# Chlumsky/msdfgen

Hardware: AMD Instinct MI355X
Metric: MSDF glyphs/sec (64x64, fp32) (higher is better)
Workload: dtype f64

## Files before the change

### msdfgen_amd/csrc/msdf_ec_fast.hpp

```cpp
#pragma once

#include "msdf_ec.hpp"

namespace msdfhip {

enum { EC_DEFER = 0x80 };

enum { EC_V_ERROR = 1,
       EC_V_CHECK = 2,
       EC_V_COND = 4,
       EC_V_HELD = 8 };
enum { EC_ORDER_EAGER = 0, EC_ORDER_LAZY = 1, EC_ORDER_LAZY_HELD = 2 };

MSDF_HD bool ecHasBasePass(const EcParams &p) { return p.distanceCheck == EC_DO_NOT_CHECK || (p.distanceCheck == EC_CHECK_AT_EDGE && p.mode != EC_MODE_EDGE_ONLY); }
MSDF_HD bool ecHasShapePass(const EcParams &p) { return p.distanceCheck == EC_ALWAYS_CHECK || p.distanceCheck == EC_CHECK_AT_EDGE; }
MSDF_HD bool ecLazyProtect(const EcParams &p) { return p.mode == EC_MODE_EDGE_PRIORITY && p.distanceCheck == EC_CHECK_AT_EDGE; }

struct FastCtx {
    double span;
    bool p1;
    bool pShape;
    bool basePass, shapePass;
    int order;
};

MSDF_HD int rangeTest2(const FastCtx &c, double at, double bt, double xt, float am, float bm, float xm) {
    const bool inversion = (am > .5f && bm > .5f && xm <= .5f) || (am < .5f && bm < .5f && xm >= .5f);
    const bool outside = medianf(am, bm, xm) != xm;
    const bool candBase = c.basePass && (inversion || (!c.p1 && outside));
    const bool candShape = c.shapePass && (inversion || (!c.pShape && outside));
    const bool candCond = c.order != EC_ORDER_EAGER && !inversion && outside;
    if (!(candBase || candShape || candCond))
        return 0;
    const double axSpan = (xt-at)*c.span, bxSpan = (bt-xt)*c.span;
    const int f = (xm >= am-axSpan && xm <= am+axSpan && xm >= bm-bxSpan && xm <= bm+bxSpan) ? 1 : 3;
    return (candBase ? f : 0)|(candShape ? f<<2 : 0)|(candCond && f == 3 ? 16 : 0);
}

MSDF_HD int judge(int flags) {
    const int cond = (flags&16) ? EC_V_COND : 0;
    if (flags&2)
        return EC_V_ERROR|cond;
    const int fs = (flags>>2)&3;
    if (fs&1)
        return ((fs&2) ? EC_V_ERROR : EC_V_CHECK)|cond;
    return cond;
}

MSDF_HD bool quadraticMayHaveRootInRange(double a, double b, double c) {
    if (a == 0 || fabs(b) > 1e12*fabs(a))
        return true;
    const double lo = .005, hi = .995;
    const double mag = fabs(a)+fabs(b)+fabs(c);
    const double eps = 1e-9*mag;
    const double flo = (a*lo+b)*lo+c, fhi = (a*hi+b)*hi+c;
    if (!(flo > eps && fhi > eps) && !(flo < -eps && fhi < -eps))
        return true;
    const double s = flo > 0 ? 1. : -1.;
    const double as = a*s, bs = b*s, cs = c*s;
    if (as <= 0)
        return false;
    if (!(-bs > 2*as*lo*(1-1e-9) && -bs < 2*as*hi*(1+1e-9)))
        return false;
    return !(4*as*cs-bs*bs > 1e-9*mag*mag);
}

MSDF_HD bool bernsteinMayHaveRoot(float dA, float dBC, float dD) {
    const float m = fmaxf(fmaxf(fabsf(dA), fabsf(dBC)), fabsf(dD));
    const float eps = 1e-5f*m;
    const float h = .5f*dBC;
    return !((dA > eps && h > eps && dD > eps) || (dA < -eps && h < -eps && dD < -eps));
}

MSDF_HD bool edgeBetweenTexelsChannelFast(const float *a, const float *b, int channel) {
    const double n = a[channel]-.5;
    const double d = a[channel]-b[channel];
    if (!((n > 0 && d > 0 && n < d) || (n < 0 && d < 0 && n > d)))
        return false;
    const double t = n/d;
    if (t > 0 && t < 1) {
        float c[3] = { mixf(a[0], b[0], t), mixf(a[1], b[1], t), mixf(a[2], b[2], t) };
        return medianf(c[0], c[1], c[2]) == c[channel];
    }
    return false;
}

MSDF_HD int edgeBetweenTexelsFast(const float *a, const float *b) {
    return 1*(int) edgeBetweenTexelsChannelFast(a, b, 0)+2*(int) edgeBetweenTexelsChannelFast(a, b, 1)+4*(int) edgeBetweenTexelsChannelFast(a, b, 2);
}

template <class Sink>
MSDF_HD int diagonalPairFast(const FastCtx &cx, float am, float dm, const float *a, const float *l, const float *q,
                             float dA, float dBC, float dD, float l0, float q0, float l1, float q1, Sink &sink) {
    const double qa = dD-dBC+dA, qb = dBC-dA-dA, qc = dA;
    if (!quadraticMayHaveRootInRange(qa, qb, qc))
        return 0;
    double t[2];
    const int solutions = solveQuadratic(t, qa, qb, qc);
    int verdict = 0;
    for (int i = 0; i < solutions; ++i) {
        if (t[i] > MSDF_ARTIFACT_T_EPSILON && t[i] < 1-MSDF_ARTIFACT_T_EPSILON) {
            const float xm = interpolatedMedianQuad(a, l, q, t[i]);
            int rangeFlags = rangeTest2(cx, 0, 1, t[i], am, dm, xm);
            const double tEx0 = -.5*l0/q0, tEx1 = -.5*l1/q1;
            if (tEx0 > 0 && tEx0 < 1) {
                double tEnd0 = 0, tEnd1 = 1;
                float em0 = am, em1 = dm;
                const float ex = interpolatedMedianQuad(a, l, q, tEx0);
                if (tEx0 > t[i])
                    tEnd1 = tEx0, em1 = ex;
                else
                    tEnd0 = tEx0, em0 = ex;
                rangeFlags |= rangeTest2(cx, tEnd0, tEnd1, t[i], em0, em1, xm);
            }
            if (tEx1 > 0 && tEx1 < 1) {
                double tEnd0 = 0, tEnd1 = 1;
                float em0 = am, em1 = dm;
                const float ex = interpolatedMedianQuad(a, l, q, tEx1);
                if (tEx1 > t[i])
                    tEnd1 = tEx1, em1 = ex;
                else
                    tEnd0 = tEx1, em0 = ex;
                rangeFlags |= rangeTest2(cx, tEnd0, tEnd1, t[i], em0, em1, xm);
            }
            const int v = judge(rangeFlags);
            verdict |= v;
            if (v&EC_V_CHECK) {
                const bool held = (verdict&EC_V_COND) != 0;
                if (held)
                    verdict |= EC_V_HELD;
                if (held == (cx.order == EC_ORDER_LAZY_HELD))
                    sink(t[i]);
            }
            if (verdict&EC_V_ERROR)
                return verdict;
        }
    }
    return verdict;
}

struct Neighbourhood {
    float v[3][3][3];
    float dev[3][3];
    unsigned valid;
};

MSDF_HD float ecTexelDeviation(const float *t) { return fabsf(medianf(t[0], t[1], t[2])-.5f); }

MSDF_HD void loadNeighbourhood(Neighbourhood &nb, const SdfView &sdf, int x, int yn) {
    nb.valid = 0;
    MSDF_UNROLL
    for (int dy = -1; dy <= 1; ++dy) {
        MSDF_UNROLL
        for (int dx = -1; dx <= 1; ++dx) {
            const int nx = x+dx, ny = yn+dy;
            const bool in = nx >= 0 && ny >= 0 && nx < sdf.w && ny < sdf.h;
            const float *t = sdf.native(in ? nx : x, in ? ny : yn);
            nb.v[dy+1][dx+1][0] = t[0], nb.v[dy+1][dx+1][1] = t[1], nb.v[dy+1][dx+1][2] = t[2];
            nb.dev[dy+1][dx+1] = ecTexelDeviation(t);
            if (in)
                nb.valid |= 1u<<((dy+1)*3+(dx+1));
        }
    }
}

template <class Emit>
MSDF_HD void texelProtectPairs(const Neighbourhood &nb, const EcParams &p, Emit &emit) {
    const float sdev = nb.dev[1][1];
    MSDF_UNROLL
    for (int dy = -1; dy <= 1; ++dy) {
        MSDF_UNROLL
        for (int dx = -1; dx <= 1; ++dx) {
            if (!dx && !dy)
                continue;
            if (!(nb.valid&(1u<<((dy+1)*3+(dx+1)))))
                continue;
            const float radius = dy == 0 ? p.radiusH : dx == 0 ? p.radiusV : p.radiusD;
            const float odev = nb.dev[dy+1][dx+1];
            const bool selfIsA = dy > 0 || (dy == 0 && dx > 0);
            const float sum = selfIsA ? sdev+odev : odev+sdev;
            if (sum < radius)
                emit((dy+1)*3+(dx+1));
        }
    }
}

MSDF_HD bool evaluateProtectPair(const float *self, const float *other, int m) {
    const int dy = m/3-1, dx = m%3-1;
    const bool selfIsA = dy > 0 || (dy == 0 && dx > 0);
    const int mask = selfIsA ? edgeBetweenTexelsFast(self, other) : edgeBetweenTexelsFast(other, self);
    return extremeChannelInMask(self, medianf(self[0], self[1], self[2]), mask);
}

MSDF_HD bool protectedByEdgesNb(const Neighbourhood &nb, const EcParams &p) {
    struct Items {
        unsigned char m[8];
        int n;
        MSDF_HD void operator()(int mm) { m[n++] = (unsigned char) mm; }
    } items;
    items.n = 0;
    texelProtectPairs(nb, p, items);
    for (int i = 0; i < items.n; ++i)
        if (evaluateProtectPair(nb.v[1][1], nb.v[items.m[i]/3][items.m[i]%3], items.m[i]))
            return true;
    return false;
}

MSDF_HD int ecNeighbourDx(int k) { return k < 4 ? (k == 0 ? -1 : k == 2 ? 1 : 0) : ((k&1) ? 1 : -1); }
MSDF_HD int ecNeighbourDy(int k) { return k < 4 ? (k == 1 ? -1 : k == 3 ? 1 : 0) : ((k&2) ? 1 : -1); }

template <class Emit>
MSDF_HD void texelCandidatePairs(const Neighbourhood &nb, Emit &emit) {
    const float *c = nb.v[1][1];
    const float cdev = nb.dev[1][1];
    MSDF_UNROLL
    for (int k = 0; k < 4; ++k) {
        const int dx = k == 0 ? -1 : k == 2 ? 1 : 0, dy = k == 1 ? -1 : k == 3 ? 1 : 0;
        if (!(nb.valid&(1u<<((dy+1)*3+(dx+1)))))
            continue;
        const float *b = nb.v[dy+1][dx+1];
        if (!(cdev >= nb.dev[dy+1][dx+1]))
            continue;
        MSDF_UNROLL
        for (int j = 0; j < 3; ++j) {
            const int i0 = j, i1 = j == 2 ? 0 : j+1;
            const float dA = c[i1]-c[i0], dB = b[i1]-b[i0];
            if ((dA > 0 && dB < 0) || (dA < 0 && dB > 0))
                emit(k, j);
        }
    }
    MSDF_UNROLL
    for (int k = 4; k < 8; ++k) {
        const int dx = (k&1) ? 1 : -1, dy = (k&2) ? 1 : -1;
        if (!(nb.valid&(1u<<((dy+1)*3+(dx+1)))))
            continue;
        const float *d = nb.v[dy+1][dx+1];
        if (!(cdev >= nb.dev[dy+1][dx+1]))
            continue;
        const float *b = nb.v[1][dx+1], *cc = nb.v[dy+1][1];
        MSDF_UNROLL
        for (int j = 0; j < 3; ++j) {
            const int i0 = j, i1 = j == 2 ? 0 : j+1;
            const float dA = c[i1]-c[i0], dBC = b[i1]-b[i0]+cc[i1]-cc[i0], dD = d[i1]-d[i0];
            if (dA == 0 && dBC == 0 && dD == 0)
                continue;
            if (bernsteinMayHaveRoot(dA, dBC, dD))
                emit(k, j);
        }
    }
}

MSDF_HD float pick3(const float *v, int i) { return i == 0 ? v[0] : i == 1 ? v[1] : v[2]; }

template <class Sink>
MSDF_HD int evaluatePair(const float *c, const float *n, const float *hb, const float *vc, const EcParams &p, bool p1, int flip, int k, int j, Sink &sink,
                         int order = EC_ORDER_EAGER) {
    FastCtx cx;
    cx.basePass = ecHasBasePass(p);
    cx.shapePass = ecHasShapePass(p);
    cx.order = order;
    cx.p1 = order != EC_ORDER_EAGER || p1;
    cx.pShape = (p.distanceCheck == EC_CHECK_AT_EDGE) ? true : cx.p1;
    const int dx = ecNeighbourDx(k), dy = ecNeighbourDy(k);
    const int i0 = j, i1 = j == 2 ? 0 : j+1;
    const float cm = medianf(c[0], c[1], c[2]), nm = medianf(n[0], n[1], n[2]);
    if (k < 4) {
        if (order == EC_ORDER_LAZY_HELD)
            return 0;
        cx.span = dy == 0 ? p.hSpan : p.vSpan;
        const float dA = pick3(c, i1)-pick3(c, i0), dB = pick3(n, i1)-pick3(n, i0);
        const double t = (double) dA/(dA-dB);
        if (t > MSDF_ARTIFACT_T_EPSILON && t < 1-MSDF_ARTIFACT_T_EPSILON) {
            const float xm = interpolatedMedianLin(c, n, t);
            const int v = judge(rangeTest2(cx, 0, 1, t, cm, nm, xm));
            if (v&EC_V_CHECK)
                sink(t, dx, flip ? -dy : dy);
            return v;
        }
        return 0;
    }
    cx.span = p.dSpan;
    const float *a = c, *b = hb, *cc = vc, *d = n;
    const float abc[3] = { a[0]-b[0]-cc[0], a[1]-b[1]-cc[1], a[2]-b[2]-cc[2] };
    const float l[3] = { -a[0]-abc[0], -a[1]-abc[1], -a[2]-abc[2] };
    const float q[3] = { d[0]+abc[0], d[1]+abc[1], d[2]+abc[2] };
    const float a3[3] = { a[0], a[1], a[2] };
    struct DirSink {
        Sink &sink;
        int dx, dy;
        MSDF_HD void operator()(double t) { sink(t, dx, dy); }
    } dirSink = { sink, dx, flip ? -dy : dy };
    const float dA = pick3(a, i1)-pick3(a, i0), dBC = pick3(b, i1)-pick3(b, i0)+pick3(cc, i1)-pick3(cc, i0), dD = pick3(d, i1)-pick3(d, i0);
    return diagonalPairFast(cx, cm, nm, a3, l, q, dA, dBC, dD, pick3(l, i0), pick3(q, i0), pick3(l, i1), pick3(q, i1), dirSink);
}

template <class Sink>
MSDF_HD int texelFindFast(const Neighbourhood &nb, const EcParams &p, bool p1, int flip, Sink &sink, int order = EC_ORDER_EAGER) {
    struct Items {
        unsigned char k[24], j[24];
        int n;
        MSDF_HD void operator()(int kk, int jj) { k[n] = (unsigned char) kk, j[n] = (unsigned char) jj; ++n; }
    } items;
    items.n = 0;
    texelCandidatePairs(nb, items);
    int verdict = 0;
    for (int i = 0; i < items.n; ++i) {
        const int k = items.k[i], dx = ecNeighbourDx(k), dy = ecNeighbourDy(k);
        verdict |= evaluatePair(nb.v[1][1], nb.v[dy+1][dx+1], nb.v[1][dx+1], nb.v[dy+1][1], p, p1, flip, k, items.j[i], sink, order);
    }
    return verdict;
}

MSDF_HD bool protectedByCornerList(const int *corners, int nCorners, int x, int ys) {
    for (int i = 0; i < nCorners; ++i) {
        const int l = corners[2*i], b = corners[2*i+1];
        if ((x == l || x == l+1) && (ys == b || ys == b+1))
            return true;
    }
    return false;
}

MSDF_HD bool ecNeedsProtection(int verdict) { return ((verdict&EC_V_COND) && !(verdict&EC_V_ERROR)) || (verdict&EC_V_HELD); }

template <class Sink>
MSDF_HD int ecTexelFast(const SdfView &sdf, const EcParams &p, const int *corners, int nCorners, int x, int yn, Sink &sink, bool allowLazy = true) {
    const int ys = sdf.flip ? sdf.h-1-yn : yn;
    Neighbourhood nb;
    loadNeighbourhood(nb, sdf, x, yn);
    int st = 0, verdict;
    if (allowLazy && ecLazyProtect(p)) {
        verdict = texelFindFast(nb, p, true, sdf.flip, sink, EC_ORDER_LAZY);
        if (ecNeedsProtection(verdict)) {
            if (!(protectedByCornerList(corners, nCorners, x, ys) || protectedByEdgesNb(nb, p)))
                verdict |= EC_V_ERROR;
            else if (verdict&EC_V_HELD)
                texelFindFast(nb, p, true, sdf.flip, sink, EC_ORDER_LAZY_HELD);
        }
    } else {
        if (p.mode == EC_MODE_EDGE_PRIORITY) {
            if (protectedByCornerList(corners, nCorners, x, ys) || protectedByEdgesNb(nb, p))
                st |= EC_PROTECTED;
        } else if (p.mode == EC_MODE_EDGE_ONLY)
            st |= EC_PROTECTED;
        verdict = texelFindFast(nb, p, (st&EC_PROTECTED) != 0, sdf.flip, sink);
    }
    if (ecHasBasePass(p) && p.distanceCheck == EC_CHECK_AT_EDGE)
        st |= EC_PROTECTED;
    if (verdict&EC_V_ERROR)
        st |= EC_ERROR;
    else if (verdict&EC_V_CHECK)
        st |= EC_DEFER;
    return st;
}

template <class Query>
MSDF_HD bool ecEvaluateCandidate(const SdfView &sdf, const EcParams &p, int x, int ys, double t, int dx, int dy, const Query &query) {
    const float *msd = sdf.shape(x, ys);
    const V2 tVector = t*mk(dx, dy);
    float oldMSD[3], newMSD[3];
    interpolate3(oldMSD, sdf, mk(x+.5, ys+.5)+tVector);
    const double aWeight = (1-fabs(tVector.x))*(1-fabs(tVector.y));
    const float aPSD = medianf(msd[0], msd[1], msd[2]);
    newMSD[0] = (float) (oldMSD[0]+aWeight*(aPSD-msd[0]));
    newMSD[1] = (float) (oldMSD[1]+aWeight*(aPSD-msd[1]));
    newMSD[2] = (float) (oldMSD[2]+aWeight*(aPSD-msd[2]));
    const float oldPSD = medianf(oldMSD[0], oldMSD[1], oldMSD[2]);
    const float newPSD = medianf(newMSD[0], newMSD[1], newMSD[2]);
    const V2 q = unproject(p.t, mk(x+.5, ys+.5))+mk(tVector.x*p.texelX, tVector.y*p.texelY);
    const float refPSD = mapDistance(p.t, query(q));
    return p.minImproveRatio*fabsf(newPSD-refPSD) < (double) fabsf(oldPSD-refPSD);
}

}
```

### msdfgen_amd/csrc/msdf_kernels.hpp

```cpp
#pragma once

#include <hip/hip_runtime.h>
#include "msdf_device.hpp"
#include "msdf_prep.hpp"
#include "msdf_ec.hpp"
#include "msdf_ec_fast.hpp"
#include "msdf_cull.hpp"
#include "msdf_scanline.hpp"
#include "msdf_shapeprep.hpp"
#include "msdf_frame.hpp"
#include "msdf_legacy.hpp"
#include "../../include/msdfgen_hip.h"

namespace msdfhip {

#ifndef MSDF_DISTANCE_WAVES_PER_SIMD
#define MSDF_DISTANCE_WAVES_PER_SIMD 4
#endif
constexpr int TILE = 8;
constexpr int WAVE = 64;
constexpr int REC_DOUBLES = sizeof(EdgeRec)/sizeof(double);

struct BatchView {
    int nGlyphs;
// ... 762 lines not shown
    __device__ double operator()(V2 q) const {
        double out[1];
        Edges edges;
        edges.coff = coff;
        if (OVERLAP)
            shapeDistanceOverlap<2>(rec, edges, windings, C, q, res, WAVE, out);
        else
            shapeDistanceSimple<2>(rec, edges, C, q, out);
        return out[0];
    }
};

typedef PB PBSlot;

struct EdgesCooperative {
    const int32_t *coff;
    int lane;
    PBSlot *slots;
    PBSlot *merged;
    int nE, C;
    mutable unsigned long long cached;
    int cacheCap;
#if defined(MSDF_PROFILE_QUERY)
    mutable unsigned long long prof[16];
#endif
    MSDF_HD int begin(int c) const { return coff[c]-coff[0]; }
    MSDF_HD int end(int c) const { return coff[c+1]-coff[0]; }
};
#if defined(MSDF_PROFILE_QUERY)
__device__ inline unsigned long long qNow() {
#if MSDF_PROFILE_QUERY >= 2
    asm volatile("s_waitcnt vmcnt(0) lgkmcnt(0)" ::: "memory");
#endif
    return __builtin_readcyclecounter();
}
__device__ inline void profAdd(const EdgesCooperative &edges, int i, unsigned long long dt) { edges.prof[i] += dt; }
__device__ inline unsigned long long profNow(const EdgesCooperative &) { return qNow(); }
__device__ unsigned long long gQueryDetail[16];
#endif

__device__ inline void selAddContour(Selector<2> &sel, const EdgeRec *rec, const EdgesCooperative &edges, int c, V2 o) {
    if (edges.slots) {
        if (c == 0) {
#if defined(MSDF_PROFILE_QUERY)
            const unsigned long long qa = qNow();
#endif
            for (int base = 0; base < edges.nE; base += WAVE) {
                const int i = base+edges.lane;
                if (i < edges.nE) {
                    Selector<2> mine;
                    selInit(mine);
                    const EdgeRegs r = loadEdgeRegs(rec+i, i);
                    selAddEdge(mine, r, i, o);
                    edges.slots[i] = mine.c[0];
                }
            }
            waveSync();
#if defined(MSDF_PROFILE_QUERY)
            const unsigned long long qb = qNow();
            edges.prof[0] += qb-qa;
#endif
            for (int cc = edges.lane; cc < edges.C; cc += WAVE) {
                PB acc;
                pbInit(acc);
                const int e = edges.end(cc);
                for (int i = edges.begin(cc); i < e; ++i) {
                    const PBSlot one = edges.slots[i];
                    pbMerge(acc, one);
                }
                edges.merged[cc] = acc;
            }
            waveSync();
#if defined(MSDF_PROFILE_QUERY)
            edges.prof[1] += qNow()-qb;
#endif
        }
        const PBSlot whole = edges.merged[c];
        pbMerge(sel.c[0], whole);
        return;
    }
    const bool cacheable = c < 64 && c < edges.cacheCap;
    if (cacheable && ((edges.cached>>c)&1ull)) {
        const PBSlot whole = edges.merged[c];
        pbMerge(sel.c[0], whole);
        return;
    }
    PB contour;
    pbInit(contour);
    const int e = edges.end(c);
    for (int base = edges.begin(c); base < e; base += WAVE) {
        Selector<2> mine;
        selInit(mine);
        const int i = base+edges.lane;
        if (i < e) {
            const EdgeRegs r = loadEdgeRegs(rec+i, i);
            selAddEdge(mine, r, i, o);
        }
        PB &m = mine.c[0];
        MSDF_UNROLL
        for (int off = 1; off < WAVE; off <<= 1) {
            PB other;
            other.td = __shfl_down(m.td, off), other.tdot = __shfl_down(m.tdot, off), other.perp = __shfl_down(m.perp, off);
            other.neg = __shfl_down(m.neg, off), other.pos = __shfl_down(m.pos, off);
            if (edges.lane+off < WAVE)
                pbMerge(m, other);
        }
        PB all;
        all.td = __shfl(m.td, 0), all.tdot = __shfl(m.tdot, 0), all.perp = __shfl(m.perp, 0), all.neg = __shfl(m.neg, 0), all.pos = __shfl(m.pos, 0);
        pbMerge(contour, all);
    }
    pbMerge(sel.c[0], contour);
    if (cacheable) {
        edges.merged[c] = contour;
        edges.cached |= 1ull<<c;
        waveSync();
    }
}

template <bool OVERLAP, class Wind = const int8_t *>
struct PsdfQueryCooperative {
    const EdgeRec *rec;
    const int32_t *coff;
    Wind windings;
    int C, lane;
    double *res;
    PBSlot *slots, *merged;
    int cacheCap = 0;
    __device__ double operator()(V2 q) const {
        double out[1];
        EdgesCooperative edges;
        edges.coff = coff, edges.lane = lane, edges.slots = slots, edges.merged = merged, edges.nE = coff[C]-coff[0], edges.C = C;
        edges.cached = 0, edges.cacheCap = slots ? 0 : cacheCap;
#if defined(MSDF_PROFILE_QUERY)
        for (int i = 0; i < 16; ++i)
            edges.prof[i] = 0;
        const unsigned long long qq0 = qNow();
#endif
        if (slots)
            waveSync();
        if (OVERLAP)
            shapeDistanceOverlap<2>(rec, edges, windings, C, q, res, 1, out);
        else
            shapeDistanceSimple<2>(rec, edges, C, q, out);
#if defined(MSDF_PROFILE_QUERY)
        if (lane == 0) {
            atomicAdd(&gQueryDetail[0], 1ull), atomicAdd(&gQueryDetail[1], qNow()-qq0);
            atomicAdd(&gQueryDetail[2], edges.prof[0]), atomicAdd(&gQueryDetail[3], edges.prof[1]), atomicAdd(&gQueryDetail[4], edges.prof[8]);
            atomicAdd(&gQueryDetail[5], edges.prof[9]), atomicAdd(&gQueryDetail[6], edges.prof[10]), atomicAdd(&gQueryDetail[7], edges.prof[11]);
            atomicAdd(&gQueryDetail[8], (unsigned long long) C), atomicAdd(&gQueryDetail[9], (unsigned long long) (slots ? 1 : 0));
        }
#endif
        return out[0];
    }
};

struct EcCandidate {
    unsigned texel;
    int dir;
    double t;
};
static_assert(sizeof(EcCandidate) == 16, "EcCandidate layout");

MSDF_HD size_t ecHeaderRecords(int nGlyphs) { return ((size_t) (nGlyphs+1)*sizeof(unsigned)+sizeof(EcCandidate)-1)/sizeof(EcCandidate); }
MSDF_HD unsigned ecSegment(size_t texelsPerGlyph) { return (unsigned) (texelsPerGlyph/8 > 64 ? (texelsPerGlyph/8+63)/64*64 : 64); }

struct CandidateSink {
    unsigned *header;
    EcCandidate *segment;
    unsigned seg, texel;
    int g;
    __device__ void operator()(double t, int dx, int dy) {
        const unsigned slot = atomicAdd(&header[1+g], 1u);
        if (slot < seg) {
            EcCandidate c;
            c.texel = texel, c.dir = (dx+1)|((dy+1)<<2), c.t = t;
            segment[slot] = c;
        } else
            header[0] = 1u;
    }
};

MSDF_HD size_t stencilIndex(size_t texel, int yn, int width, int height, int stencilYDown) {
    return stencilYDown ? texel+(size_t) (height-1-2*yn)*width : texel;
}

struct EcGlyphParams {
    double hSpan, vSpan, dSpan, texelX, texelY;
    float radiusH, radiusV, radiusD;
    int cornerBegin, nCorners;
    int pad;
};
static_assert(sizeof(EcGlyphParams) == 64, "EcGlyphParams layout");

__device__ __forceinline__ void ecParamsBody(EcGlyphParams *out, const BatchView &batch, const MsdfHipGlyph *glyphs, const MsdfHipConfig &cfg, unsigned *candidateHeader,
                                             int *corners, int *sizes, const int g, const int lane) {
    if (candidateHeader && lane == 0) {
        candidateHeader[1+g] = 0;
        if (g == 0)
            candidateHeader[0] = 0;
    }
    EcParams p;
    p.t = loadXform(glyphs[g]);
    p.minDeviationRatio = cfg.min_deviation_ratio;
    p.minImproveRatio = cfg.min_improve_ratio;
    ecDerive(p);
    const int c0 = batch.glyphContourOffsets[g], C = batch.glyphContourOffsets[g+1]-c0;
    const int e0 = batch.contourOffsets[c0], nE = batch.contourOffsets[c0+C]-e0;
    int nCorners = 0;
    if (cfg.ec_mode == EC_MODE_EDGE_PRIORITY && corners) {
        const EdgeRec *rec = batch.recs+e0;
        for (int base = 0; base < nE; base += WAVE) {
            const int e = base+lane;
            const bool corner = e < nE && (rec[e].flags&REC_CORNER);
            const unsigned long long mask = __ballot(corner);
            if (corner) {
                const V2 pp = project(p.t, ld(rec[e].p0));
                const int slot = e0+nCorners+__popcll(mask&((1ull<<lane)-1ull));
                corners[2*slot] = (int) floor(pp.x-.5);
                corners[2*slot+1] = (int) floor(pp.y-.5);
            }
            nCorners += __popcll(mask);
        }
    }
    if (lane == 0) {
        EcGlyphParams o;
        o.hSpan = p.hSpan, o.vSpan = p.vSpan, o.dSpan = p.dSpan, o.texelX = p.texelX, o.texelY = p.texelY;
        o.radiusH = p.radiusH, o.radiusV = p.radiusV, o.radiusD = p.radiusD, o.cornerBegin = e0, o.nCorners = nCorners, o.pad = 0;
        out[g] = o;
        if (sizes)
            sizes[2*g] = nE, sizes[2*g+1] = C;
    }
}
__global__ void __launch_bounds__(WAVE)
k_ec_params(EcGlyphParams *out, BatchView batch, const MsdfHipGlyph *glyphs, MsdfHipConfig cfg, unsigned *candidateHeader, int *corners, int *sizes) {
    ecParamsBody(out, batch, glyphs, cfg, candidateHeader, corners, sizes, (int) blockIdx.x, (int) threadIdx.x);
}

#ifndef MSDF_EC_FAST_WAVES_PER_SIMD
#define MSDF_EC_FAST_WAVES_PER_SIMD 7
#endif
enum { EC_HALO = TILE+2, EC_QUEUE_CAP = WAVE*24, EC_PROTECT_QUEUE_CAP = WAVE*8 };
__host__ __device__ inline size_t ecFastLdsBytes(int maxEdges, int n) {
    return (size_t) EC_HALO*EC_HALO*n*sizeof(float)+(WAVE+4)*sizeof(int)
           +(EC_QUEUE_CAP+EC_PROTECT_QUEUE_CAP)*sizeof(unsigned short);
}

__device__ __forceinline__ bool ecTileCornerTexel(const int *list, int nCorners, int tx, int ty, int height, int flip, int lane) {
    const int lxT = lane&(TILE-1), lyT = lane>>3;
    const int xT = tx*TILE+lxT, ysT = flip ? height-1-(ty*TILE+lyT) : ty*TILE+lyT;
    const int x0 = tx*TILE, x1 = tx*TILE+TILE-1;
    const int ya = flip ? height-1-(ty*TILE+TILE-1) : ty*TILE, yb = flip ? height-1-ty*TILE : ty*TILE+TILE-1;
    bool cornerTexel = false;
    for (int base = 0; base < nCorners; base += WAVE) {
        const int k = base+lane;
        int l = 0, b = 0;
        bool near = false;
        if (k < nCorners) {
            l = list[2*k], b = list[2*k+1];
            near = l+1 >= x0 && l <= x1 && b+1 >= ya && b <= yb;
        }
        for (unsigned long long mask = __ballot(near); mask; mask &= mask-1) {
            const int src = __ffsll((long long) mask)-1;
            const int cl = __builtin_amdgcn_readlane(l, src), cb = __builtin_amdgcn_readlane(b, src);
            cornerTexel = cornerTexel || ((xT == cl || xT == cl+1) && (ysT == cb || ysT == cb+1));
        }
    }
    return cornerTexel;
}

template <int N>
__device__ __forceinline__ void ecRunProtectQueue(const float *halo, const unsigned short *protectQueue, int nProtect, int *verdictLds, int lane) {
    for (int base = 0; base < nProtect; base += WAVE) {
        const int it = base+lane;
        if (it >= nProtect)
            continue;
        const unsigned item = protectQueue[it];
        const int s = item&63, m = item>>6;
        const int sx = s&(TILE-1), sy = s>>3;
        const float *self = halo+((sy+1)*EC_HALO+sx+1)*N, *other = halo+((sy+m/3)*EC_HALO+sx+m%3)*N;
        if (evaluateProtectPair(self, other, m))
            atomicOr(&verdictLds[s], 0x100);
    }
}

struct EcPushProtect {
    unsigned short *queue;
    int *count;
    int lane;
    __device__ void operator()(int m) { queue[atomicAdd(count, 1)] = (unsigned short) (lane|m<<6); }
};

template <int N, int ORDER = -1>
__device__ __forceinline__ void ecFastBody(const BatchView &batch, const MsdfHipGlyph *glyphs, int width, int height, int tilesX, int tilesPerGlyph,
          const float *src, float *out, uint8_t *stencilOut, const MsdfHipConfig &cfg, const EcGlyphParams *glyphParams, EcCandidate *cands, unsigned seg,
          int maxEdges, const int *corners, const unsigned blockId, int *smemFast, const int sinkSlots = 0, const int sinkSlot = 0) {
    const GlyphWork wk = decodeItem(blockId, batch.nGlyphs, tilesPerGlyph);
    if (!wk.valid)
        return;
    float *halo = reinterpret_cast<float *>(smemFast);
    int *verdictLds = reinterpret_cast<int *>(halo+EC_HALO*EC_HALO*N);
    int *itemCount = verdictLds+WAVE;
    unsigned short *queue = reinterpret_cast<unsigned short *>(itemCount+4);
    unsigned short *protectQueue = queue+EC_QUEUE_CAP;
    float *devLds = reinterpret_cast<float *>(queue+EC_QUEUE_CAP)-EC_HALO*EC_HALO;
    static_assert((EC_QUEUE_CAP*sizeof(unsigned short))%sizeof(float) == 0 && EC_QUEUE_CAP*sizeof(unsigned short) >= EC_HALO*EC_HALO*sizeof(float), "devLds overlays the queue's tail");
    const int lane = threadIdx.x;
    const MsdfHipGlyph gd = glyphs[wk.g];
    EcParams p;
    p.t = loadXform(gd);
    p.minDeviationRatio = cfg.min_deviation_ratio;
    p.minImproveRatio = cfg.min_improve_ratio;
    p.mode = cfg.ec_mode, p.distanceCheck = cfg.ec_distance_check, p.overlap = cfg.overlap_support, p.stageLimit = 0;
    const EcGlyphParams gp = glyphParams[wk.g];
    p.hSpan = gp.hSpan, p.vSpan = gp.vSpan, p.dSpan = gp.dSpan, p.texelX = gp.texelX, p.texelY = gp.texelY;
    p.radiusH = gp.radiusH, p.radiusV = gp.radiusV, p.radiusD = gp.radiusD;
    const int tx = wk.tile%tilesX, ty = wk.tile/tilesX;

    const bool lazy = ORDER < 0 ? ecLazyProtect(p) : ORDER != 0;
    bool cornerTexel = false;
    if (p.mode == EC_MODE_EDGE_PRIORITY && !lazy)
        cornerTexel = ecTileCornerTexel(corners+2*(size_t) gp.cornerBegin, gp.nCorners, tx, ty, height, gd.flip, lane);

    const float *field = src+(size_t) wk.g*height*width*N;
    for (int idx = lane; idx < EC_HALO*EC_HALO; idx += WAVE) {
        const int hx = tx*TILE+idx%EC_HALO-1, hy = ty*TILE+idx/EC_HALO-1;
        if (hx >= 0 && hy >= 0 && hx < width && hy < height) {
            const float *t = field+((size_t) hy*width+hx)*N;
            float tv[N];
            for (int ch = 0; ch < N; ++ch)
                tv[ch] = t[ch], halo[idx*N+ch] = tv[ch];
            devLds[idx] = ecTexelDeviation(tv);
        }
    }
    if (lane < 2)
        itemCount[lane] = 0;
    waveSync();

    const int lx = lane&(TILE-1), ly = lane>>3;
    const int x = tx*TILE+lx, yn = ty*TILE+ly;
    const bool inside = x < width && yn < height;
    int st = 0;
    const bool classify = inside;
    Neighbourhood nb;
    nb.valid = 0;
    if (classify) {
        MSDF_UNROLL
        for (int dy = -1; dy <= 1; ++dy) {
            MSDF_UNROLL
            for (int dx = -1; dx <= 1; ++dx) {
                const int nx = x+dx, ny = yn+dy;
                const bool in = nx >= 0 && ny >= 0 && nx < width && ny < height;
                const float *t = halo+((ly+1+(in ? dy : 0))*EC_HALO+lx+1+(in ? dx : 0))*N;
                nb.v[dy+1][dx+1][0] = t[0], nb.v[dy+1][dx+1][1] = t[1], nb.v[dy+1][dx+1][2] = t[2];
                nb.dev[dy+1][dx+1] = devLds[(ly+1+(in ? dy : 0))*EC_HALO+lx+1+(in ? dx : 0)];
                if (in)
                    nb.valid |= 1u<<((dy+1)*3+(dx+1));
            }
        }
    }
    waveSync();
    if (classify) {
        if (p.mode == EC_MODE_EDGE_PRIORITY && !lazy) {
            if (cornerTexel)
                st |= EC_PROTECTED;
            if (!(st&EC_PROTECTED)) {
                EcPushProtect pushProtect = { protectQueue, itemCount+1, lane };
                texelProtectPairs(nb, p, pushProtect);
            }
        } else if (p.mode == EC_MODE_EDGE_ONLY)
            st |= EC_PROTECTED;
        struct Push {
            unsigned short *queue;
            int *count;
            int lane;
            __device__ void operator()(int k, int j) { queue[atomicAdd(count, 1)] = (unsigned short) (lane|k<<6|j<<9); }
        } push = { queue, itemCount, lane };
        texelCandidatePairs(nb, push);
    }
    verdictLds[lane] = (st&EC_PROTECTED) ? 0x100 : 0;
    waveSync();

    if (!lazy) {
        ecRunProtectQueue<N>(halo, protectQueue, itemCount[1], verdictLds, lane);
        waveSync();
    }

    const int nItems = itemCount[0];
    const auto runItems = [&](const int order) {
        for (int base = 0; base < nItems; base += WAVE) {
            const int it = base+lane;
            if (it >= nItems)
                continue;
            const unsigned item = queue[it];
            const int s = item&63, k = (item>>6)&7, jp = item>>9;
            const int word = verdictLds[s];
            if (order == EC_ORDER_LAZY_HELD && (word&(0x100|EC_V_HELD)) != (0x100|EC_V_HELD))
                continue;
            const int sx = s&(TILE-1), sy = s>>3;
            const int dx = ecNeighbourDx(k), dy = ecNeighbourDy(k);
            const float *c = halo+((sy+1)*EC_HALO+sx+1)*N, *n = halo+((sy+1+dy)*EC_HALO+sx+1+dx)*N;
            const float *hb = halo+((sy+1)*EC_HALO+sx+1+dx)*N, *vc = halo+((sy+1+dy)*EC_HALO+sx+1)*N;
            CandidateSink sink;
            sink.header = reinterpret_cast<unsigned *>(cands);
            sink.segment = sinkSlots > 0 ? cands+ecHeaderRecords(sinkSlots)+(size_t) sinkSlot*seg : cands+ecHeaderRecords(batch.nGlyphs)+(size_t) wk.g*seg;
            sink.seg = seg, sink.g = sinkSlots > 0 ? sinkSlot : wk.g;
            sink.texel = (unsigned) (((size_t) wk.g*height+ty*TILE+sy)*width+tx*TILE+sx);
            const int v = evaluatePair(c, n, hb, vc, p, (word&0x100) != 0, gd.flip, k, jp, sink, order);
            if (v && order != EC_ORDER_LAZY_HELD)
                atomicOr(&verdictLds[s], v);
        }
    };
    runItems(lazy ? EC_ORDER_LAZY : EC_ORDER_EAGER);
    waveSync();

    const bool need = lazy && inside && ecNeedsProtection(verdictLds[lane]);
    if (__ballot(need)) {
        __asm__ volatile("" ::: "memory");
        const EcGlyphParams gl = glyphParams[wk.g];
        EcParams pr = p;
        pr.radiusH = gl.radiusH, pr.radiusV = gl.radiusV, pr.radiusD = gl.radiusD;
        cornerTexel = ecTileCornerTexel(corners+2*(size_t) gl.cornerBegin, gl.nCorners, tx, ty, height, gd.flip, lane);
        if (need) {
            if (cornerTexel)
                verdictLds[lane] |= 0x100;
            else {
                Neighbourhood nd;
                nd.valid = 0;
                MSDF_UNROLL
                for (int dy = -1; dy <= 1; ++dy) {
                    MSDF_UNROLL
                    for (int dx = -1; dx <= 1; ++dx) {
                        const int nx = x+dx, ny = yn+dy;
                        const bool in = nx >= 0 && ny >= 0 && nx < width && ny < height;
                        nd.dev[dy+1][dx+1] = ecTexelDeviation(halo+((ly+1+(in ? dy : 0))*EC_HALO+lx+1+(in ? dx : 0))*N);
                        if (in)
                            nd.valid |= 1u<<((dy+1)*3+(dx+1));
                    }
                }
                EcPushProtect pushProtect = { protectQueue, itemCount+1, lane };
                texelProtectPairs(nd, pr, pushProtect);
            }
        }
        waveSync();
        ecRunProtectQueue<N>(halo, protectQueue, itemCount[1], verdictLds, lane);
        waveSync();
        bool revisit = false;
        if (need) {
            const int word = verdictLds[lane];
            if (!(word&0x100))
                verdictLds[lane] = word|EC_V_ERROR;
            revisit = (word&0x100) && (word&EC_V_HELD);
        }
        if (__ballot(revisit)) {
            waveSync();
            runItems(EC_ORDER_LAZY_HELD);
        }
    }

    if (!inside)
        return;
    const int verdict = verdictLds[lane];
    if ((verdict&0x100) || (ecHasBasePass(p) && p.distanceCheck == EC_CHECK_AT_EDGE))
        st |= EC_PROTECTED;
    if (verdict&EC_V_ERROR)
        st |= EC_ERROR;
    const size_t texel = ((size_t) wk.g*height+yn)*width+x;
    const float *in = halo+((ly+1)*EC_HALO+lx+1)*N;
    float v[N];
    for (int i = 0; i < N; ++i)
        v[i] = in[i];
    if (st&EC_ERROR) {
        const float m = medianf(v[0], v[1], v[2]);
        v[0] = m, v[1] = m, v[2] = m;
    }
    float *px = out+gd.out_offset+(ptrdiff_t) gd.row_stride*yn+(ptrdiff_t) N*x;
    for (int i = 0; i < N; ++i)
        px[i] = v[i];
    if (stencilOut)
        stencilOut[stencilIndex(texel, yn, width, height, cfg.stencil_y_down)] = (uint8_t) st;
}
template <int N, bool LAZY>
__global__ void __launch_bounds__(WAVE, MSDF_EC_FAST_WAVES_PER_SIMD)
k_ec_fast(BatchView batch, const MsdfHipGlyph *glyphs, int width, int height, int tilesX, int tilesPerGlyph,
          const float *src, float *out, uint8_t *stencilOut, MsdfHipConfig cfg, const EcGlyphParams *glyphParams, EcCandidate *cands, unsigned seg,
          int maxEdges, const int *corners) {
    extern __shared__ int smemFast[];
    ecFastBody<N, LAZY ? 1 : 0>(batch, glyphs, width, height, tilesX, tilesPerGlyph, src, out, stencilOut, cfg, glyphParams, cands, seg, maxEdges, corners, blockIdx.x, smemFast);
}

struct EcQueryPolicy { int lpcMaxContours, lpcEdgeCost, lpcMaxEdges, lpcMinCount, wideMaxEdges; float wideLoad, wideMeanCount; int gridSteps; };
MSDF_HD int ecQueryGridSlices(unsigned count, int nE, int C, EcQueryPolicy q) {
    if (q.gridSteps <= 0 || C > q.lpcMaxContours || count == 0)
        return 0;
    int J = 1;
    while (J < (int) count && J < WAVE)
        J <<= 1;
    int S = WAVE/J, need = 1;
    while (need*q.gridSteps < nE && need < WAVE)
        need <<= 1;
    if (need > S)
        S = need;
    return S >= 2 && S <= WAVE/2 ? S : 0;
}
MSDF_HD bool ecQueryLanePerCandidate(unsigned count, int nE, int C, EcQueryPolicy q) {
    if (C > q.lpcMaxContours)
        return false;
    if ((nE > q.lpcMaxEdges && (int) count < q.lpcMinCount))
        return false;
    const long long coop = (long long) count*(340ll*((nE+WAVE-1)/WAVE)+10ll*nE+1000ll);
    const long long lpc = (long long) ((count+WAVE-1)/WAVE)*((long long) q.lpcEdgeCost*nE+1000ll);
    return lpc < coop;
}
MSDF_HD int ecQueryItems(unsigned count, unsigned seg, int nE, int C, EcQueryPolicy lpcMaxContours) {
    if (count > seg)
        return 0;
    const int S = ecQueryGridSlices(count, nE, C, lpcMaxContours);
    if (S)
        return (int) ((count+WAVE/S-1)/(WAVE/S));
    return ecQueryLanePerCandidate(count, nE, C, lpcMaxContours) ? (int) ((count+WAVE-1)/WAVE) : (int) count;
}
MSDF_HD bool ecQueryListedFirst(unsigned count, int nE, int C, EcQueryPolicy q) {
    return ecQueryGridSlices(count, nE, C, q) != 0 || ecQueryLanePerCandidate(count, nE, C, q) || (q.gridSteps > 0 && nE > WAVE);
}

MSDF_HD size_t ecQueuesAt(int nGlyphs) { return 2*((size_t) nGlyphs+1)+2+2*(size_t) nGlyphs; }
MSDF_HD size_t ecOffsetInts(int nGlyphs) { return ecQueuesAt(nGlyphs)+8*16; }
MSDF_HD size_t ecSizesAt(int nGlyphs) { return 2*((size_t) nGlyphs+1)+2; }

__global__ void __launch_bounds__(1024)
k_ec_scan(int nGlyphs, const unsigned *__restrict__ header, unsigned seg, int *__restrict__ offsets, EcQueryPolicy lpcMaxContours, const int *__restrict__ order) {
    __shared__ int waveTotals[2][16];
    __shared__ float waveLoad[16], waveCount[16];
    enum { PER = 8 };
    const int t = threadIdx.x, lane = t&(WAVE-1), wave = t/WAVE;
    const int *sizes = offsets+ecSizesAt(nGlyphs);
    float mine = 0, mineCount = 0;
    for (int base = 0; base < nGlyphs; base += 1024*PER) {
        unsigned count[PER];
        int nE[PER];
        MSDF_UNROLL
        for (int k = 0; k < PER; ++k) {
            const int p = base+t*PER+k;
            const int g = p < nGlyphs ? (order ? order[p] : p) : -1;
            count[k] = g >= 0 ? header[1+g] : 0u, nE[k] = g >= 0 ? sizes[2*g] : 0;
        }
        MSDF_UNROLL
        for (int k = 0; k < PER; ++k)
            if (count[k] <= seg)
                mine += (float) count[k]*(340.f*((nE[k]+WAVE-1)/WAVE)+10.f*nE[k]+1000.f), mineCount += (float) count[k];
    }
    for (int off = WAVE/2; off > 0; off >>= 1)
        mine += __shfl_down(mine, off), mineCount += __shfl_down(mineCount, off);
    if (lane == 0)
        waveLoad[wave] = mine, waveCount[wave] = mineCount;
    __syncthreads();
    float total = 0, totalCount = 0;
    for (int w = 0; w < 16; ++w)
        total += waveLoad[w], totalCount += waveCount[w];
    const bool dense = lpcMaxContours.wideMeanCount > 0 && totalCount >= lpcMaxContours.wideMeanCount*(float) nGlyphs;
    if ((total > lpcMaxContours.wideLoad || dense) && lpcMaxContours.wideMaxEdges > lpcMaxContours.lpcMaxEdges)
        lpcMaxContours.lpcMaxEdges = lpcMaxContours.wideMaxEdges;
    const bool gridOff = total > lpcMaxContours.wideLoad || dense || lpcMaxContours.gridSteps <= 0;
    if (gridOff)
        lpcMaxContours.gridSteps = 0;
    int *coop = offsets+nGlyphs+1;
    int carry[2] = { 0, 0 };
    for (int base = 0; base < nGlyphs; base += 1024*PER) {
        int items[PER];
        bool chunky[PER];
        int sum[2] = { 0, 0 };
        MSDF_UNROLL
        for (int k = 0; k < PER; ++k) {
            const int p = base+t*PER+k;
            const int g = p < nGlyphs ? (order ? order[p] : p) : -1;
            const unsigned count = g >= 0 ? header[1+g] : 0u;
            const int nE = g >= 0 ? sizes[2*g] : 0, C = g >= 0 ? sizes[2*g+1] : 0;
            chunky[k] = g >= 0 && ecQueryListedFirst(count, nE, C, lpcMaxContours);
            items[k] = g >= 0 ? ecQueryItems(count, seg, nE, C, lpcMaxContours) : 0;
            sum[chunky[k] ? 0 : 1] += items[k];
        }
        int incl[2] = { sum[0], sum[1] };
        for (int off = 1; off < WAVE; off <<= 1) {
            const int n0 = __shfl_up(incl[0], off), n1 = __shfl_up(incl[1], off);
            if (lane >= off)
                incl[0] += n0, incl[1] += n1;
        }
        if (lane == WAVE-1)
            waveTotals[0][wave] = incl[0], waveTotals[1][wave] = incl[1];
        __syncthreads();
        int before[2] = { 0, 0 }, all[2] = { 0, 0 };
        for (int w = 0; w < 16; ++w) {
            const int v0 = waveTotals[0][w], v1 = waveTotals[1][w];
            if (w < wave)
                before[0] += v0, before[1] += v1;
            all[0] += v0, all[1] += v1;
        }
        int at[2] = { carry[0]+before[0]+incl[0]-sum[0], carry[1]+before[1]+incl[1]-sum[1] };
        MSDF_UNROLL
        for (int k = 0; k < PER; ++k) {
            const int p = base+t*PER+k;
            if (p < nGlyphs) {
                offsets[p] = at[0], coop[p] = at[1];
                at[chunky[k] ? 0 : 1] += items[k];
            }
        }
        carry[0] += all[0], carry[1] += all[1];
        __syncthreads();
    }
    if (t == 1023) {
        offsets[nGlyphs] = carry[0];
        coop[nGlyphs] = carry[1];
        coop[nGlyphs+1] = 0;
        for (int q = 0; q < 8; ++q)
            offsets[ecQueuesAt(nGlyphs)+16*q] = 0;
        coop[nGlyphs+2] = lpcMaxContours.lpcMaxEdges|(gridOff ? 1<<30 : 0);
    }
}

#ifndef MSDF_EC_QUERY_WAVES_PER_SIMD
#define MSDF_EC_QUERY_WAVES_PER_SIMD 3
#endif
#if defined(MSDF_PROFILE_QUERY)
__device__ unsigned long long gQueryProfile[24];
#if MSDF_PROFILE_QUERY >= 2
#define MSDF_QSTAMP(x) asm volatile("s_waitcnt vmcnt(0) lgkmcnt(0)" ::: "memory"); const unsigned long long x = __builtin_readcyclecounter()
#else
#define MSDF_QSTAMP(x) const unsigned long long x = __builtin_readcyclecounter()
#endif
#endif
template <int N, bool OVERLAP>
__global__ void __launch_bounds__(WAVE, MSDF_EC_QUERY_WAVES_PER_SIMD)
k_ec_query(int nGlyphs, const int32_t *__restrict__ glyphContourOffsets, const int32_t *__restrict__ contourOffsets, const EdgeRec *__restrict__ recs,
           const int8_t *__restrict__ windings, const MsdfHipGlyph *__restrict__ glyphs, int width, int height, const float *__restrict__ src, float *__restrict__ out,
           uint8_t *__restrict__ stencilOut, MsdfHipConfig cfg, const EcGlyphParams *__restrict__ glyphParams, const EcCandidate *__restrict__ cands, unsigned seg,
           const int *__restrict__ offsets, int *__restrict__ counter, int itemsPerTicket, int slotCap, int slotOffset, EcQueryPolicy lpcMaxContours,
           unsigned *__restrict__ overflowOut, const int *__restrict__ order, int queryFlags) {
    if (overflowOut && blockIdx.x == 0 && threadIdx.x == 0)
        *overflowOut = reinterpret_cast<const unsigned *>(cands)[0];
    BatchView batch;
    batch.nGlyphs = nGlyphs, batch.glyphContourOffsets = glyphContourOffsets, batch.contourOffsets = contourOffsets, batch.recs = recs, batch.windings = windings;
    extern __shared__ double smemLds[];
    PBSlot *slotBuf = reinterpret_cast<PBSlot *>(smemLds+slotOffset);
    const unsigned *header = reinterpret_cast<const unsigned *>(cands);
    const size_t texelsPerGlyph = (size_t) width*height;
    const int chunks = offsets[batch.nGlyphs], coopItems = offsets[2*batch.nGlyphs+1];
    const int tickets = chunks+(coopItems+itemsPerTicket-1)/itemsPerTicket;
    lpcMaxContours.lpcMaxEdges = offsets[2*batch.nGlyphs+3]&((1<<30)-1);
    if (offsets[2*batch.nGlyphs+3]&(1<<30))
        lpcMaxContours.gridSteps = 0;
#if defined(MSDF_PROFILE_QUERY)
    MSDF_QSTAMP(qStart);
    unsigned long long qAcc[8] = { 0, 0, 0, 0, 0, 0, 0, 0 }, qItems[4] = { 0, 0, 0, 0 }, qLongest = 0, qLastWork = 0, qLongestWho = 0;
#endif
    const int dealt = (queryFlags&1) ? (int) gridDim.x : 0;
    for (int round = 0;; ++round) {
#if defined(MSDF_PROFILE_QUERY)
        MSDF_QSTAMP(q0);
#endif
        int ticket = 0;
        if (dealt && (queryFlags&4) && round > 0) {
            const int q = (int) blockIdx.x&7;
            if (threadIdx.x == 0)
                ticket = atomicAdd(counter+(ecQueuesAt(batch.nGlyphs)-(2*(size_t) batch.nGlyphs+2))+16*q, 1);
            ticket = dealt+__builtin_amdgcn_readfirstlane(ticket)*8+q;
            if (ticket >= tickets)
                break;
        } else if (dealt) {
            if ((long long) round*dealt >= tickets)
                break;
            ticket = (round&1) ? (round+1)*dealt-1-(int) blockIdx.x : round*dealt+(int) blockIdx.x;
            if (ticket >= tickets)
                continue;
        } else {
            if (threadIdx.x == 0)
                ticket = atomicAdd(counter, 1);
            ticket = __builtin_amdgcn_readfirstlane(ticket);
            if (ticket >= tickets)
                break;
        }
#if defined(MSDF_PROFILE_QUERY)
        MSDF_QSTAMP(q1);
        qAcc[0] += q1-q0;
#endif
        const int *part = ticket < chunks ? offsets : offsets+batch.nGlyphs+1;
        const int first = ticket < chunks ? ticket : (ticket-chunks)*itemsPerTicket;
        const int last = ticket < chunks ? first+1 : (first+itemsPerTicket < coopItems ? first+itemsPerTicket : coopItems);
        int lo = 0, hi = batch.nGlyphs-1;
        while (lo < hi) {
            const int mid = (lo+hi)>>1;
            if (part[mid+1] > first)
                hi = mid;
            else
                lo = mid+1;
        }
        int pos = lo;
        MSDF_NOUNROLL
        for (int i = first; i < last; ++i) {
#if defined(MSDF_PROFILE_QUERY)
        MSDF_QSTAMP(q2a);
#endif
        while (part[pos+1] <= i)
            ++pos;
        const int item = i-part[pos];
        const int g = order ? order[pos] : pos;
#if defined(MSDF_PROFILE_QUERY)
        MSDF_QSTAMP(q2);
        qAcc[1] += q2-(i == first ? q1 : q2a);
#endif
        const unsigned count = header[1+g];
        const EcCandidate *segment = cands+ecHeaderRecords(batch.nGlyphs)+(size_t) g*seg;
        const int c0 = batch.glyphContourOffsets[g], C = batch.glyphContourOffsets[g+1]-c0;
        const int32_t *coff = batch.contourOffsets+c0;
        const MsdfHipGlyph gd = glyphs[g];
        EcParams p;
        p.t = loadXform(gd);
        p.minDeviationRatio = cfg.min_deviation_ratio;
        p.minImproveRatio = cfg.min_improve_ratio;
        p.mode = cfg.ec_mode, p.distanceCheck = cfg.ec_distance_check, p.overlap = OVERLAP, p.stageLimit = 0;
        const EcGlyphParams gp = glyphParams[g];
        p.hSpan = gp.hSpan, p.vSpan = gp.vSpan, p.dSpan = gp.dSpan, p.texelX = gp.texelX, p.texelY = gp.texelY;
        p.radiusH = gp.radiusH, p.radiusV = gp.radiusV, p.radiusD = gp.radiusD;
        SdfView sdf;
        sdf.px = src+(size_t) g*texelsPerGlyph*N;
        sdf.w = width, sdf.h = height, sdf.N = N, sdf.flip = gd.flip;
        const int nE = coff[C]-coff[0];
        WindingMasks wind;
        wind.mem = batch.windings+c0;
        wind.pos = wind.neg = 0;
        if (OVERLAP) {
            const int w = (int) threadIdx.x < C ? (int) wind.mem[threadIdx.x] : 0;
            wind.pos = __ballot(w > 0), wind.neg = __ballot(w < 0);
        }
#if defined(MSDF_PROFILE_QUERY)
        MSDF_QSTAMP(q3);
        qAcc[2] += q3-q2;
        unsigned long long q4 = q3;
        const bool qChunk = ecQueryListedFirst(count, nE, C, lpcMaxContours);
#endif
        const int gridS = ecQueryGridSlices(count, nE, C, lpcMaxContours);
// ... 652 lines not shown
```

Baseline: 1.826 million.

## Precompute per-texel channel-gradient sign words in LDS for EC candidate tests

During halo staging, each texel now gets a packed class word holding the sign of each channel difference plus an inside flag. It is stored next to its deviation in LDS, and the halo load is unrolled into two fixed rounds with strength-reduced addressing. Candidate pair detection then uses bitwise ops on these words instead of recomputing float differences per neighbour, and the in-bounds mask comes from the inside flag. This cuts repeated arithmetic and branching in the classify phase. In exchange it adds LDS footprint in the queue overlay and reads neighbour class words unconditionally before the sync.

```diff
diff --git a/msdfgen_amd/csrc/msdf_ec_fast.hpp b/msdfgen_amd/csrc/msdf_ec_fast.hpp
--- a/msdfgen_amd/csrc/msdf_ec_fast.hpp
+++ b/msdfgen_amd/csrc/msdf_ec_fast.hpp
@@ -142,13 +142,32 @@
 struct Neighbourhood {
     float v[3][3][3];
     float dev[3][3];
+    unsigned cls[3][3];
     unsigned valid;
 };
 
 MSDF_HD float ecTexelDeviation(const float *t) { return fabsf(medianf(t[0], t[1], t[2])-.5f); }
 
+enum { EC_CLS_INSIDE = 0x8000 };
+MSDF_HD unsigned ecTexelClassWord(const float *t) {
+    unsigned w = EC_CLS_INSIDE;
+    MSDF_UNROLL
+    for (int j = 0; j < 3; ++j) {
+        const float d = t[j == 2 ? 0 : j+1]-t[j];
+        w |= (d > 0 ? 1u<<j : 0u)|(d < 0 ? 8u<<j : 0u)|(d == 0 ? 64u<<j : 0u);
+    }
+    return w;
+}
+
+MSDF_HD unsigned ecValidFromWords(const Neighbourhood &nb) {
+    unsigned valid = 0;
+    MSDF_UNROLL
+    for (int m = 0; m < 9; ++m)
+        valid |= (nb.cls[m/3][m%3]&EC_CLS_INSIDE) ? 1u<<m : 0u;
+    return valid;
+}
+
 MSDF_HD void loadNeighbourhood(Neighbourhood &nb, const SdfView &sdf, int x, int yn) {
-    nb.valid = 0;
     MSDF_UNROLL
     for (int dy = -1; dy <= 1; ++dy) {
         MSDF_UNROLL
@@ -158,10 +177,10 @@
             const float *t = sdf.native(in ? nx : x, in ? ny : yn);
             nb.v[dy+1][dx+1][0] = t[0], nb.v[dy+1][dx+1][1] = t[1], nb.v[dy+1][dx+1][2] = t[2];
             nb.dev[dy+1][dx+1] = ecTexelDeviation(t);
-            if (in)
-                nb.valid |= 1u<<((dy+1)*3+(dx+1));
-        }
-    }
+            nb.cls[dy+1][dx+1] = in ? ecTexelClassWord(t) : 0u;
+        }
+    }
+    nb.valid = ecValidFromWords(nb);
 }
 
 template <class Emit>
@@ -173,7 +192,7 @@
         for (int dx = -1; dx <= 1; ++dx) {
             if (!dx && !dy)
                 continue;
-            if (!(nb.valid&(1u<<((dy+1)*3+(dx+1)))))
+            if (!(nb.cls[dy+1][dx+1]&EC_CLS_INSIDE))
                 continue;
             const float radius = dy == 0 ? p.radiusH : dx == 0 ? p.radiusV : p.radiusD;
             const float odev = nb.dev[dy+1][dx+1];
@@ -213,36 +232,36 @@
 MSDF_HD void texelCandidatePairs(const Neighbourhood &nb, Emit &emit) {
     const float *c = nb.v[1][1];
     const float cdev = nb.dev[1][1];
+    const unsigned cw = nb.cls[1][1];
     MSDF_UNROLL
     for (int k = 0; k < 4; ++k) {
         const int dx = k == 0 ? -1 : k == 2 ? 1 : 0, dy = k == 1 ? -1 : k == 3 ? 1 : 0;
-        if (!(nb.valid&(1u<<((dy+1)*3+(dx+1)))))
-            continue;
-        const float *b = nb.v[dy+1][dx+1];
-        if (!(cdev >= nb.dev[dy+1][dx+1]))
-            continue;
-        MSDF_UNROLL
-        for (int j = 0; j < 3; ++j) {
-            const int i0 = j, i1 = j == 2 ? 0 : j+1;
-            const float dA = c[i1]-c[i0], dB = b[i1]-b[i0];
-            if ((dA > 0 && dB < 0) || (dA < 0 && dB > 0))
-                emit(k, j);
+        const unsigned nw = nb.cls[dy+1][dx+1];
+        const unsigned opposite = ((cw&(nw>>3))|((cw>>3)&nw))&7u;
+        const unsigned m = cdev >= nb.dev[dy+1][dx+1] ? opposite : 0u;
+        if (m) {
+            if (m&1u)
+                emit(k, 0);
+            if (m&2u)
+                emit(k, 1);
+            if (m&4u)
+                emit(k, 2);
         }
     }
     MSDF_UNROLL
     for (int k = 4; k < 8; ++k) {
         const int dx = (k&1) ? 1 : -1, dy = (k&2) ? 1 : -1;
-        if (!(nb.valid&(1u<<((dy+1)*3+(dx+1)))))
+        const unsigned dw = nb.cls[dy+1][dx+1];
+        if (!(((dw&EC_CLS_INSIDE) != 0)&(cdev >= nb.dev[dy+1][dx+1])))
             continue;
         const float *d = nb.v[dy+1][dx+1];
-        if (!(cdev >= nb.dev[dy+1][dx+1]))
-            continue;
         const float *b = nb.v[1][dx+1], *cc = nb.v[dy+1][1];
+        const unsigned zeroAD = cw&dw;
         MSDF_UNROLL
         for (int j = 0; j < 3; ++j) {
             const int i0 = j, i1 = j == 2 ? 0 : j+1;
             const float dA = c[i1]-c[i0], dBC = b[i1]-b[i0]+cc[i1]-cc[i0], dD = d[i1]-d[i0];
-            if (dA == 0 && dBC == 0 && dD == 0)
+            if ((zeroAD&(64u<<j)) && dBC == 0)
                 continue;
             if (bernsteinMayHaveRoot(dA, dBC, dD))
                 emit(k, j);
diff --git a/msdfgen_amd/csrc/msdf_kernels.hpp b/msdfgen_amd/csrc/msdf_kernels.hpp
--- a/msdfgen_amd/csrc/msdf_kernels.hpp
+++ b/msdfgen_amd/csrc/msdf_kernels.hpp
@@ -1088,8 +1088,13 @@
     int *itemCount = verdictLds+WAVE;
     unsigned short *queue = reinterpret_cast<unsigned short *>(itemCount+4);
     unsigned short *protectQueue = queue+EC_QUEUE_CAP;
-    float *devLds = reinterpret_cast<float *>(queue+EC_QUEUE_CAP)-EC_HALO*EC_HALO;
-    static_assert((EC_QUEUE_CAP*sizeof(unsigned short))%sizeof(float) == 0 && EC_QUEUE_CAP*sizeof(unsigned short) >= EC_HALO*EC_HALO*sizeof(float), "devLds overlays the queue's tail");
+    struct TexelClass {
+        float dev;
+        unsigned cls;
+    };
+    TexelClass *classLds = reinterpret_cast<TexelClass *>(queue+EC_QUEUE_CAP)-EC_HALO*EC_HALO;
+    static_assert((EC_QUEUE_CAP*sizeof(unsigned short))%sizeof(TexelClass) == 0 && EC_QUEUE_CAP*sizeof(unsigned short) >= EC_HALO*EC_HALO*sizeof(TexelClass)
+                  && 2*WAVE >= EC_HALO*EC_HALO && WAVE%EC_HALO == 4 && WAVE/EC_HALO == 6, "classLds overlays the queue's tail; the halo is staged in two rounds");
     const int lane = threadIdx.x;
     const MsdfHipGlyph gd = glyphs[wk.g];
     EcParams p;
@@ -1107,15 +1112,28 @@
     if (p.mode == EC_MODE_EDGE_PRIORITY && !lazy)
         cornerTexel = ecTileCornerTexel(corners+2*(size_t) gp.cornerBegin, gp.nCorners, tx, ty, height, gd.flip, lane);
 
-    const float *field = src+(size_t) wk.g*height*width*N;
-    for (int idx = lane; idx < EC_HALO*EC_HALO; idx += WAVE) {
-        const int hx = tx*TILE+idx%EC_HALO-1, hy = ty*TILE+idx/EC_HALO-1;
-        if (hx >= 0 && hy >= 0 && hx < width && hy < height) {
-            const float *t = field+((size_t) hy*width+hx)*N;
-            float tv[N];
-            for (int ch = 0; ch < N; ++ch)
-                tv[ch] = t[ch], halo[idx*N+ch] = tv[ch];
-            devLds[idx] = ecTexelDeviation(tv);
+    const ptrdiff_t rowStep = (ptrdiff_t) width*N;
+    const ptrdiff_t origin = (((ptrdiff_t) wk.g*height+ty*TILE-1)*width+tx*TILE-1)*N;
+    const int hr0 = lane/EC_HALO, hc0 = lane-hr0*EC_HALO;
+    const ptrdiff_t laneStep0 = hr0*rowStep+hc0*N;
+    MSDF_UNROLL
+    for (int round = 0; round < 2; ++round) {
+        const int idx = lane+round*WAVE;
+        const bool wrap = round && hc0+WAVE%EC_HALO >= EC_HALO;
+        const int hc = hc0+round*(WAVE%EC_HALO)-(wrap ? EC_HALO : 0), hr = hr0+round*(WAVE/EC_HALO)+(wrap ? 1 : 0);
+        const ptrdiff_t laneStep = laneStep0+round*((WAVE/EC_HALO)*rowStep+(WAVE%EC_HALO)*N)+(wrap ? rowStep-EC_HALO*N : 0);
+        if (idx < EC_HALO*EC_HALO) {
+            const int hx = tx*TILE+hc-1, hy = ty*TILE+hr-1;
+            unsigned cls = 0;
+            if (hx >= 0 && hy >= 0 && hx < width && hy < height) {
+                const float *t = src+(origin+laneStep);
+                float tv[N];
+                for (int ch = 0; ch < N; ++ch)
+                    tv[ch] = t[ch], halo[idx*N+ch] = tv[ch];
+                classLds[idx].dev = ecTexelDeviation(tv);
+                cls = ecTexelClassWord(tv);
+            }
+            classLds[idx].cls = cls;
         }
     }
     if (lane < 2)
@@ -1128,24 +1146,25 @@
     int st = 0;
     const bool classify = inside;
     Neighbourhood nb;
-    nb.valid = 0;
+    const int centre = (ly+1)*EC_HALO+lx+1;
+    MSDF_UNROLL
+    for (int dy = -1; dy <= 1; ++dy) {
+        MSDF_UNROLL
+        for (int dx = -1; dx <= 1; ++dx) {
+            const TexelClass tc = classLds[centre+dy*EC_HALO+dx];
+            nb.dev[dy+1][dx+1] = tc.dev, nb.cls[dy+1][dx+1] = tc.cls;
+        }
+    }
+    waveSync();
     if (classify) {
         MSDF_UNROLL
         for (int dy = -1; dy <= 1; ++dy) {
             MSDF_UNROLL
             for (int dx = -1; dx <= 1; ++dx) {
-                const int nx = x+dx, ny = yn+dy;
-                const bool in = nx >= 0 && ny >= 0 && nx < width && ny < height;
-                const float *t = halo+((ly+1+(in ? dy : 0))*EC_HALO+lx+1+(in ? dx : 0))*N;
+                const float *t = halo+(centre+dy*EC_HALO+dx)*N;
                 nb.v[dy+1][dx+1][0] = t[0], nb.v[dy+1][dx+1][1] = t[1], nb.v[dy+1][dx+1][2] = t[2];
-                nb.dev[dy+1][dx+1] = devLds[(ly+1+(in ? dy : 0))*EC_HALO+lx+1+(in ? dx : 0)];
-                if (in)
-                    nb.valid |= 1u<<((dy+1)*3+(dx+1));
-            }
-        }
-    }
-    waveSync();
-    if (classify) {
+            }
+        }
         if (p.mode == EC_MODE_EDGE_PRIORITY && !lazy) {
             if (cornerTexel)
                 st |= EC_PROTECTED;
@@ -1211,7 +1230,6 @@
                 verdictLds[lane] |= 0x100;
             else {
                 Neighbourhood nd;
-                nd.valid = 0;
                 MSDF_UNROLL
                 for (int dy = -1; dy <= 1; ++dy) {
                     MSDF_UNROLL
@@ -1219,8 +1237,7 @@
                         const int nx = x+dx, ny = yn+dy;
                         const bool in = nx >= 0 && ny >= 0 && nx < width && ny < height;
                         nd.dev[dy+1][dx+1] = ecTexelDeviation(halo+((ly+1+(in ? dy : 0))*EC_HALO+lx+1+(in ? dx : 0))*N);
-                        if (in)
-                            nd.valid |= 1u<<((dy+1)*3+(dx+1));
+                        nd.cls[dy+1][dx+1] = in ? (unsigned) EC_CLS_INSIDE : 0u;
                     }
                 }
                 EcPushProtect pushProtect = { protectQueue, itemCount+1, lane };
```

New measurement: 1.858 million, median of 6. +1.7%, better.
